# plancherb1/parallel-DDP

Measured on AMD Instinct MI355X. Metric: DDP iterations/sec (Kuka iiwa14 N=128, 8 alphas, 4 shooting segments), higher is better.
Workload: dtype f32; 1 GPU; BASELINE configs[2]: Kuka iiwa14 RBD (n=14,m=7), N=128, 8 alphas x 4 shooting segments, Euler, fp32, joint cost, T=0.5 s, WAFR example inputs + N(0,1e-3) velocity noise; problems_per_gpu=16384, problems_total=16384, hipgraph=True, cost_to_go_slots_written=all, handle_options=library defaults

## Files before the change

parallel-ddp_amd/csrc/pddp_tl.hip:

```cpp
#include <hip/hip_runtime.h>

#include "ab_compact.hpp"
#include "bodies.hpp"
#include "fp_lg.hpp"
#include "fp_pipe.hpp"
#include "tl_launch.hpp"

namespace pddp {

template <typename T> struct TlStagedSink {
    typedef T v4 __attribute__((ext_vector_type(4)));
    T* ds; mutable T* cur; int stride; T* stg; int lane, a, A;
    __device__ __forceinline__ void x(int, const T*) const {}
    __device__ __forceinline__ void u(int, const T*) const {}
    __device__ __forceinline__ void d(int k, const T* v) const { tl_store14(ds + (size_t)k * 14, v); }
    __device__ __forceinline__ void xu(int, const T* xv, const T* uv) const {
        wsync();
        T* rec = stg + lane * 22;
        tl_store14(rec, xv); tl_store7(rec + 14, uv);
        wsync();
        const T* src = stg + (lane - a) * 22 + 4 * a; T* dst = cur - 18 * a;
        const int step = 4 * A;
#pragma unroll
        for (int j = 0; j < 5; j++) *reinterpret_cast<v4*>(dst + step * j) = *reinterpret_cast<const v4*>(src + step * j);
        if (2 * a < A) *reinterpret_cast<v4*>(dst + step * 5) = *reinterpret_cast<const v4*>(src + step * 5);
        cur += stride;
    }
    __device__ __forceinline__ void xu_last(int, const T* xv, const T* uv) const { tl_store14(cur, xv); tl_store7(cur + 14, uv); }
};
constexpr int kFpTlPS = 132;
constexpr int kFpTlMaxPairs = 8;
template <typename T, int V, bool ALL, bool EE = false, bool PC = false>
#ifndef PDDP_FP_TL_MINBLK
#define PDDP_FP_TL_MINBLK 3
#endif
__global__ __launch_bounds__(256, sizeof(T) == 4 && !EE && !ALL && !PC ? PDDP_FP_TL_MINBLK : 2) void k_fp_tl(Buffers<T> b, Dims dm, CostWeights<T> cw, T dt, T grav, int batch) {
    if constexpr (!PC) b.cwt = nullptr;
    constexpr ArmTlModel<T> md = arm_tl_builtin<T>(V);
    constexpr int NX = 14, NU = 7, PS = kFpTlPS;
    const int A = dm.A, M = dm.M, N = dm.N, NBk = dm.NB, per_pb = M * A, total = batch * per_pb;
    const int inst = blockIdx.x * 256 + threadIdx.x;
    if (A < 8 || (64 % A) != 0) {
        if (inst >= total) return;
        const int pb = inst / per_pb, rem = inst - pb * per_pb, seg = rem / A, a_idx = rem - seg * A;
        if (!fp_active<T>(b, dm, pb)) return;
        const T* xcur = b.xb + ((size_t)pb * 2 + b.state[pb].cur) * N * NX;
        if (EE) {
            if (ALL) arm_tl_rollout_segment_ee<T>(md, grav, b, dm, cw, dt, pb, a_idx, seg, xcur, tl_candidate_sink<T>(b, dm, pb, a_idx), true);
            else arm_tl_rollout_segment_ee<T>(md, grav, b, dm, cw, dt, pb, a_idx, seg, xcur, tl_state_sink<T>(b, dm, pb, a_idx), true);
        } else {
            if (ALL) arm_tl_rollout_segment<T>(md, grav, b, dm, cw, dt, pb, a_idx, seg, xcur, tl_candidate_sink<T>(b, dm, pb, a_idx), true);
            else arm_tl_rollout_segment<T>(md, grav, b, dm, cw, dt, pb, a_idx, seg, xcur, tl_state_sink<T>(b, dm, pb, a_idx), true);
        }
        return;
    }
    __shared__ __attribute__((aligned(16))) T stage_all[4 * 2 * kFpTlMaxPairs * PS];
    const int wave = threadIdx.x >> 6, lane = threadIdx.x & 63;
    T* stg = stage_all + wave * (2 * kFpTlMaxPairs * PS);
    const int ppw = 64 / A, npairs = batch * M;
    const int gp0 = (blockIdx.x * 256 + wave * 64) / A;
    if (gp0 >= npairs) return;
    constexpr int J2 = (kFpTlMaxPairs * 56 + 63) / 64, J1 = (kFpTlMaxPairs * 14 + 63) / 64;
    const T* src2[J2]; int dst2[J2], str2[J2];
    const T* src1[J1]; int dst1[J1];
#pragma unroll
    for (int j = 0; j < J2; j++) {
        const int e = lane + 64 * j, q = e / 56, off = e - q * 56;
        int gq = gp0 + (q < ppw ? q : ppw - 1); gq = gq < npairs ? gq : npairs - 1;
        const int pbq = gq / M, k0 = (gq - pbq * M) * NBk;
        const bool isK = off < 49;
        src2[j] = isK ? b.KT + ((size_t)pbq * N + k0) * (NX * NU) + 2 * off
                      : b.xb + (((size_t)pbq * 2 + b.state[pbq].cur) * N + k0) * NX + 2 * (off - 49);
        str2[j] = isK ? NX * NU : NX;
        dst2[j] = (e < ppw * 56) ? q * PS + (isK ? 2 * off : 98 + 2 * (off - 49)) : -1;
    }
#pragma unroll
    for (int j = 0; j < J1; j++) {
        const int e = lane + 64 * j, q = e / 14, off = e - q * 14;
        int gq = gp0 + (q < ppw ? q : ppw - 1); gq = gq < npairs ? gq : npairs - 1;
        const int pbq = gq / M, k0 = (gq - pbq * M) * NBk;
        src1[j] = (off < 7 ? b.ucur : b.du) + ((size_t)pbq * N + k0) * NU + (off < 7 ? off : off - 7);
        dst1[j] = (e < ppw * 14) ? q * PS + 112 + off : -1;
    }
    TlPair<T> pf2[J2]; T pf1[J1];
    auto fetch = [&]() {
#pragma unroll
        for (int j = 0; j < J2; j++) { pf2[j] = *reinterpret_cast<const TlPair<T>*>(src2[j]); src2[j] += str2[j]; }
#pragma unroll
        for (int j = 0; j < J1; j++) { pf1[j] = src1[j][0]; src1[j] += NU; }
    };
    auto park = [&](int buf) {
        T* d = stg + buf * (kFpTlMaxPairs * PS);
#pragma unroll
        for (int j = 0; j < J2; j++) if (dst2[j] >= 0) *reinterpret_cast<TlPair<T>*>(d + dst2[j]) = pf2[j];
#pragma unroll
        for (int j = 0; j < J1; j++) if (dst1[j] >= 0) d[dst1[j]] = pf1[j];
    };
    const int p = lane / A, a_idx = lane - p * A, gp = gp0 + p;
    const int pb = (gp < npairs ? gp : npairs - 1) / M, seg = (gp < npairs ? gp : npairs - 1) - pb * M;
    const bool live = gp < npairs && fp_active<T>(b, dm, pb);
    const T* xcur = b.xb + ((size_t)pb * 2 + b.state[pb].cur) * N * NX;
    constexpr bool REC = PC && !EE;
    constexpr int XGS = REC ? 24 : 16;
    __shared__ __attribute__((aligned(16))) T xg_all[4 * kFpTlMaxPairs * XGS];
    T* xg = xg_all + (wave * kFpTlMaxPairs + p) * XGS;
    if (a_idx == 0) { T t[NX]; tl_load14(t, b.xGoal + (size_t)pb * NX); tl_store14(xg, t); }
    if constexpr (REC) {
        if (a_idx == 0) {
            const CostWeights<T> own = cost_weights_at(b, cw, pb);
            xg[16] = own.Q1; xg[17] = own.Q2; xg[18] = own.R; xg[19] = own.QF1; xg[20] = own.QF2;
        }
    }
    const auto own_cw = [&]() { if constexpr (REC) return cost_weights_joint_row(cw, xg + 16); else return cw; };
    T xt[EE ? NX : 1], acc[EE ? NU : 1];
    int tshift = 0;
    if (EE) {
        tl_load14(xt, b.xTarget + (size_t)pb * NX);
#pragma unroll
        for (int i = 0; i < NU; i++) acc[i] = T(0);
        tshift = b.tshift[pb];
    }
    TlRollout<T> r;
    r.iters = 0;
    const auto csink = tl_candidate_sink<T>(b, dm, pb, a_idx);
    constexpr bool STG = sizeof(T) == 4 && !ALL;
    const auto rsink = tl_run_sink<T>(b, dm, pb, a_idx, seg * NBk);
    const auto ssink = [&]() { if constexpr (STG) return TlStagedSink<T>{rsink.ds, rsink.cur, rsink.stride, stg, lane, a_idx, A}; else return rsink; }();
    if (live) {
        if (ALL) tl_rollout_begin<T>(r, b, dm, pb, a_idx, seg, xcur, csink); else tl_rollout_begin<T>(r, b, dm, pb, a_idx, seg, xcur, ssink);
        if (EE) r.iters = NBk;
    }
    fetch(); park(0);
    wsync();
    for (int k = 0; k < NBk; k++) {
        if (k + 1 < NBk) fetch();
        if (live && k < r.iters) {
            const T* o = stg + (k & 1) * (kFpTlMaxPairs * PS) + p * PS;
            if (EE) {
                if (ALL) tl_rollout_step_ee<T>(r, acc, md, grav, b, dm, cw, dt, k, o, o + 98, o + 112, o + 119, xg, xt, tshift, csink);
                else tl_rollout_step_ee<T>(r, acc, md, grav, b, dm, cw, dt, k, o, o + 98, o + 112, o + 119, xg, xt, tshift, ssink);
            } else {
                if (ALL) tl_rollout_step<T>(r, md, grav, b, dm, own_cw(), dt, k, o, o + 98, o + 112, o + 119, xg, csink);
                else tl_rollout_step<T>(r, md, grav, b, dm, own_cw(), dt, k, o, o + 98, o + 112, o + 119, xg, ssink);
            }
        }
        if (k + 1 < NBk) park((k + 1) & 1);
        wsync();
    }
    if (!live) return;
    if (EE) tl_rollout_end_ee<T>(r, acc, dm);
    else {
        T ucN[NU];
#pragma unroll
        for (int i = 0; i < NU; i++) ucN[i] = b.ucur[((size_t)pb * N + (N - 1)) * NU + i];
        if (ALL) tl_rollout_end<T>(r, dm, own_cw(), ucN, xg, csink); else tl_rollout_end<T>(r, dm, own_cw(), ucN, xg, ssink);
    }
    const size_t slot = (size_t)pb * A + a_idx;
    b.Jpart[slot * M + seg] = r.J; b.dpart[slot * M + seg] = r.sdef;
    b.parts_fresh[pb] = 1;
}

template <int V>
__global__ __launch_bounds__(128, 1) void k_fp_tl2(Buffers<float> b, Dims dm, CostWeights<float> cw, float dt, float grav, int batch) {
    using T = float;
    constexpr ArmTlModel<T> md = arm_tl_builtin<T>(V);
    constexpr int NX = 14, NU = 7, ST = 9, SX = 15;
    __shared__ T s_tau[64 * ST];
    __shared__ T s_x[64 * SX];
    const int wave = __builtin_amdgcn_readfirstlane((int)threadIdx.x >> 6), lane = threadIdx.x & 63;
    const int A = dm.A, M = dm.M, N = dm.N, NBk = dm.NB, total = batch * M * A;
    const int inst_raw = blockIdx.x * 64 + lane, inst = inst_raw < total ? inst_raw : total - 1;
    const int pb = inst / (M * A), rem = inst - pb * (M * A), seg = rem / A, a_idx = rem - seg * A;
    const bool live = inst_raw < total && fp_active<T>(b, dm, pb);
    cw = cost_weights_at(b, cw, pb);
    const int kStart = seg * NBk, iters = (seg < M - 1) ? NBk : NBk - 1;
    const T* xcur = b.xb + ((size_t)pb * 2 + b.state[pb].cur) * N * NX;
    const size_t slot = (size_t)pb * A + a_idx;
    T* xs = b.xs + slot * N * NX; T* us = b.us + slot * N * NU; T* ds = b.ds + slot * N * NX;
    T x[NX];
    if (seg == 0) tl_load14(x, xcur); else tl_load14(x, xs + (size_t)kStart * NX);
    if (wave == 0) {
        const T alpha = b.alpha[a_idx];
        const T* KT = b.KT + (size_t)pb * N * NX * NU; const T* uc = b.ucur + (size_t)pb * N * NU; const T* du = b.du + (size_t)pb * N * NU;
        T xg[NX];
        tl_load14(xg, b.xGoal + (size_t)pb * NX);
        T J = T(0);
        T nK[NX * NU], nxr[NX], nuc[NU], ndu[NU];
        auto fetch = [&](int kn) {
#pragma unroll
            for (int rr = 0; rr < NU; rr++) tl_load14(nK + rr * NX, KT + (size_t)kn * (NX * NU) + rr * NX);
            tl_load14(nxr, xcur + (size_t)kn * NX);
#pragma unroll
            for (int i = 0; i < NU; i++) { nuc[i] = uc[(size_t)kn * NU + i]; ndu[i] = du[(size_t)kn * NU + i]; }
        };
        fetch(kStart);
        for (int k = 0; k < NBk; k++) {
            const int kn = kStart + k;
            const bool act = live && k < iters;
            if (act) {
                T u[NU];
                tl_control_law<T>(u, alpha, ndu, nK, x, nxr, nuc);
                if (k + 1 < NBk) fetch(kn + 1);
#pragma unroll
                for (int i = 0; i < NU; i++) us[(size_t)kn * NU + i] = u[i];
                J += arm_tl_cost<T>(cw, x, u, xg, false);
                ArmTlState<T> st;
                T bias[NU];
                arm_tl_trig<T>(st, x);
                arm_tl_bias<T>(md, grav, st, x + 7, bias);
#pragma unroll
                for (int i = 0; i < NU; i++) s_tau[lane * ST + i] = u[i] - bias[i];
            }
            __syncthreads();
            __syncthreads();
            if (act && k < NBk - 1) {
#pragma unroll
                for (int i = 0; i < NX; i++) x[i] = s_x[lane * SX + i];
            }
        }
        if (live) {
            if (seg == M - 1) {
                T u[NU];
#pragma unroll
                for (int i = 0; i < NU; i++) { u[i] = uc[(size_t)(N - 1) * NU + i]; us[(size_t)(N - 1) * NU + i] = u[i]; }
                J += arm_tl_cost<T>(cw, x, u, xg, true);
            }
            b.Jpart[slot * M + seg] = J;
            b.parts_fresh[pb] = 1;
        }
    } else {
        if (live) tl_store14(xs + (size_t)kStart * NX, x);
        T sdef = T(0);
        for (int k = 0; k < NBk; k++) {
            const int kn = kStart + k;
            const bool act = live && k < iters;
            ArmTlState<T> st;
            if (act) { arm_tl_trig<T>(st, x); arm_tl_factor<T>(md, st); }
            __syncthreads();
            if (act) {
                T qdd[NU], xn[NX];
#pragma unroll
                for (int i = 0; i < NU; i++) qdd[i] = s_tau[lane * ST + i];
                tl_ldl_solve(st, qdd);
#pragma unroll
                for (int i = 0; i < 7; i++) { xn[i] = x[i] + dt * x[7 + i]; xn[7 + i] = x[7 + i] + dt * qdd[i]; }
                if (k < NBk - 1) {
#pragma unroll
                    for (int i = 0; i < NX; i++) { x[i] = xn[i]; s_x[lane * SX + i] = xn[i]; }
                    tl_store14(xs + (size_t)(kn + 1) * NX, xn);
                } else {
                    const int ks = (seg + 1) * NBk;
                    T xnext[NX], e[NX];
                    tl_load14(xnext, xs + (size_t)ks * NX);
#pragma unroll
                    for (int i = 0; i < NX; i++) { e[i] = xn[i] - xnext[i]; sdef += tabs(e[i]); }
                    tl_store14(ds + (size_t)(ks - 1) * NX, e);
                }
            }
            __syncthreads();
        }
        if (live) b.dpart[slot * M + seg] = (seg == M - 1) ? T(0) : sdef;
    }
}
void launch_fp_tl2(hipStream_t s, int variant, const Buffers<float>& b, const Dims& dm, const CostWeights<float>& cw, float dt, float grav, int batch) {
    const unsigned inst = (unsigned)batch * dm.M * dm.A;
    if (variant == 0) hipLaunchKernelGGL((k_fp_tl2<0>), dim3((inst + 63) / 64), dim3(128), 0, s, b, dm, cw, dt, grav, batch);
    else hipLaunchKernelGGL((k_fp_tl2<1>), dim3((inst + 63) / 64), dim3(128), 0, s, b, dm, cw, dt, grav, batch);
}

template <typename T> __device__ __forceinline__ T tl4_fma(T a, T b_, T c) { return __builtin_fma(a, b_, c); }
template <> __device__ __forceinline__ float tl4_fma<float>(float a, float b_, float c) { return __builtin_fmaf(a, b_, c); }
template <typename T, int V, bool EE>
__global__ __launch_bounds__(256, 1) void k_fp_tl4(Buffers<T> b, Dims dm, CostWeights<T> cw, T dt, T grav, int batch, SolverParams sp, int ls_mode, int maps) {
    constexpr int NX = 14, NU = 7;
    __shared__ T ls_J[64], ls_d[64];
    extern __shared__ __attribute__((aligned(16))) unsigned char pipe_lds_raw[];
    const TlPipeLdsT<T> p = tl_pipe_lds(reinterpret_cast<T*>(pipe_lds_raw), true);
    const int wave = __builtin_amdgcn_readfirstlane((int)threadIdx.x >> 6), lane = threadIdx.x & 63;
    if (threadIdx.x < kPipeFlags) p.flag[threadIdx.x] = 0;
    const int A = dm.A, M = dm.M, N = dm.N, NBk = dm.NB, total = batch * M * A;
    const int inst_raw = blockIdx.x * 64 + lane, inst = inst_raw < total ? inst_raw : total - 1;
    const int pb = inst / (M * A), rem = inst - pb * (M * A), seg = rem / A, a_idx = rem - seg * A;
    const bool live = inst_raw < total && fp_active<T>(b, dm, pb);
    cw = cost_weights_at(b, cw, pb);
    const int kStart = seg * NBk;
    const T* xcur = b.xb + ((size_t)pb * 2 + b.state[pb].cur) * N * NX;
    const size_t slot = (size_t)pb * A + a_idx;
    T* xs = b.xs + slot * N * NX; T* us = b.us + slot * N * NU; T* ds = b.ds + slot * N * NX;
    const T alpha = b.alpha[a_idx];
    T x[NX];
    if (!maps) { if (seg == 0) tl_load14(x, xcur); else tl_load14(x, xs + (size_t)kStart * NX); }
    else {
        const int W = M * A, l = rem < NX ? rem : NX - 1;
        const T* dcur = b.dcur + (size_t)pb * N * NX;
        tl_load14(x, xcur + (size_t)kStart * NX);
        T es = T(0), et = T(0);
        auto advance = [&](int sgm, const T* ph, T gam, T dk) {
            T ns = gam, nt = dk;
#pragma unroll
            for (int cc = 0; cc < NX; cc++) { ns = tl4_fma<T>(ph[cc], __shfl(es, cc, W), ns); nt = tl4_fma<T>(ph[cc], __shfl(et, cc, W), nt); }
            es = ns; et = nt;
#pragma unroll
            for (int i = 0; i < NX; i++) {
                const T si = __shfl(es, i, W), ti = __shfl(et, i, W);
                if (seg == sgm + 1) x[i] = x[i] + (ti - alpha * si);
            }
        };
        if (M == 4) {
            T ph[3][NX + 1], dk[3];
#pragma unroll
            for (int sgm = 0; sgm < 3; sgm++) {
                const T* o = b.segmap + ((size_t)pb * 4 + sgm) * 256;
#pragma unroll
                for (int cc = 0; cc <= NX; cc++) ph[sgm][cc] = o[cc * 16 + l];
                dk[sgm] = dcur[(size_t)((sgm + 1) * NBk - 1) * NX + l];
            }
#pragma unroll
            for (int sgm = 0; sgm < 3; sgm++) advance(sgm, ph[sgm], ph[sgm][NX], dk[sgm]);
        } else {
            for (int sgm = 0; sgm < M - 1; sgm++) {
                const T* o = b.segmap + ((size_t)pb * M + sgm) * 256;
                T ph[NX + 1];
#pragma unroll
                for (int cc = 0; cc <= NX; cc++) ph[cc] = o[cc * 16 + l];
                advance(sgm, ph, ph[NX], dcur[(size_t)((sgm + 1) * NBk - 1) * NX + l]);
            }
        }
    }
    __syncthreads();
    if (wave >= 2) { tl_pipe_factor_wave<V>(p, wave - 2, NBk, x, dt, lane); return; }
    if (wave == 0) {
        for (int k = 0; k < NBk; k++) tl_pipe_chain_step<V, true>(p, k, x, (const T*)nullptr, dt, grav, lane);
        return;
    }
    T x0[NX];
#pragma unroll
    for (int i = 0; i < NX; i++) x0[i] = x[i];
    const T* KT = b.KT + (size_t)pb * N * NX * NU; const T* uc = b.ucur + (size_t)pb * N * NU; const T* du = b.du + (size_t)pb * N * NU;
    T xg[NX], goal[6], acc7s[NU];
    int tshift = 0;
    if (EE) {
#pragma unroll
        for (int i = 0; i < 6; i++) goal[i] = b.xGoal[(size_t)pb * NX + i];
        tl_load14(xg, b.xTarget + (size_t)pb * NX);
        tshift = b.tshift[pb];
#pragma unroll
        for (int i = 0; i < NU; i++) acc7s[i] = T(0);
    } else tl_load14(xg, b.xGoal + (size_t)pb * NX);
    T J = T(0), sdef = T(0);
    T nK[NX * NU], nxr[NX], nuc[NU], ndu[NU];
    auto fetch = [&](int kn) {
#pragma unroll
        for (int rr = 0; rr < NU; rr++) tl_load14(nK + rr * NX, KT + (size_t)kn * (NX * NU) + rr * NX);
        tl_load14(nxr, xcur + (size_t)kn * NX);
#pragma unroll
        for (int i = 0; i < NU; i++) { nuc[i] = uc[(size_t)kn * NU + i]; ndu[i] = du[(size_t)kn * NU + i]; }
    };
    fetch(kStart);
    if (live) tl_store14(xs + (size_t)kStart * NX, x);
    const int iters = EE ? NBk : ((seg < M - 1) ? NBk : NBk - 1);
    for (int k = 0; k < NBk; k++) {
        const int kn = kStart + k;
        if (k > 0) {
            T xv[16];
            tl_pipe_wait(p.flag + 0, k);
            tl_pipe_ld<4>(xv, p.xbuf + (((k & 1) * 64) + lane) * kPipeSX);
#pragma unroll
            for (int i = 0; i < NX; i++) x[i] = xv[i];
        }
        T u[8];
        tl_control_law<T>(u, alpha, ndu, nK, x, nxr, nuc);
        u[7] = T(0);
        tl_pipe_st<2>(p.ubuf + (((k & 1) * 64) + lane) * kPipeSU, u);
        tl_pipe_post(p.flag + 1, k + 1);
        if (k + 1 < NBk) fetch(kn + 1);
        if (k > 0 && live) tl_store14(xs + (size_t)kn * NX, x);
        if (live && k < iters) {
#pragma unroll
            for (int i = 0; i < NU; i++) us[(size_t)kn * NU + i] = u[i];
            if (!EE) J += arm_tl_cost<T>(cw, x, u, xg, false);
            else if (k < NBk - 1 || seg == M - 1) {
                constexpr ArmTlModel<T> md = arm_tl_builtin<T>(V);
                ArmTlState<T> st;
                arm_tl_trig<T>(st, x);
                ArmTlFrames<T> fr;
                arm_tl_world_chain<false, T>(md, st.c, st.s, fr);
                T pos[6];
                arm_tl_tool_point<T>(fr, cw.ee_z, tl_ee_rpy_weighted<T>(cw), pos);
#pragma unroll
                for (int ind = 0; ind < NU; ind++) {
                    T cost = T(0);
                    if (ind == 0) cost += ee_term<T>(cw, pos, goal, kn >= N - 1 - tshift);
                    acc7s[ind] += ee_joint_terms<T>(cw, x, u, xg, ind, kn, N, cost);
                }
            }
        }
    }
    T xnext[NX];
    if (maps) {
#pragma unroll
        for (int i = 0; i < NX; i++) xnext[i] = __shfl(x0[i], (lane + A) & 63);
    }
    if (seg < M - 1) {
        tl_pipe_wait(p.flag + 0, NBk);
        if (live) {
            T xi[16];
            tl_pipe_ld<4>(xi, p.xbuf + ((((NBk) & 1) * 64) + lane) * kPipeSX);
            const int ks = (seg + 1) * NBk;
            T e[NX];
            if (!maps) tl_load14(xnext, xs + (size_t)ks * NX);
#pragma unroll
            for (int i = 0; i < NX; i++) { e[i] = xi[i] - xnext[i]; sdef += tabs(e[i]); }
            tl_store14(ds + (size_t)(ks - 1) * NX, e);
        }
    } else if (!EE && live) {
        T u[NU];
#pragma unroll
        for (int i = 0; i < NU; i++) { u[i] = uc[(size_t)(N - 1) * NU + i]; us[(size_t)(N - 1) * NU + i] = u[i]; }
        J += arm_tl_cost<T>(cw, x, u, xg, true);
    }
    if (EE) J = acc7s[0] + acc7s[1] + acc7s[2] + acc7s[3] + acc7s[4] + acc7s[5] + acc7s[6];
    const T dseg = (seg == M - 1) ? T(0) : sdef;
    if (live) {
        b.Jpart[slot * M + seg] = J;
        b.dpart[slot * M + seg] = dseg;
        if (ls_mode < 0) b.parts_fresh[pb] = 1;
    }
    if (ls_mode >= 0) {
        ls_J[lane] = J; ls_d[lane] = dseg;
        wsync();
        const int base = lane - rem;
        if (live && seg == 0) {
            T Jt = T(0), mx = T(0);
            for (int sgm = 0; sgm < M; sgm++) { Jt += ls_J[base + sgm * A + a_idx]; mx = tmax(mx, ls_d[base + sgm * A + a_idx]); }
            b.J[slot] = Jt; b.dmax[slot] = mx;
            ls_J[lane] = Jt; ls_d[lane] = mx;
        }
        wsync();
        if (inst_raw < total && rem == 0) ls_body<T>(b, dm, sp, pb, ls_mode, ls_J + lane, ls_d + lane);
    }
}
template <typename T>
void launch_fp_tl4(hipStream_t s, int variant, const Buffers<T>& b, const Dims& dm, const CostWeights<T>& cw, T dt, T grav, int batch, const SolverParams& sp, int ls_mode, bool maps) {
    const unsigned inst = (unsigned)batch * dm.M * dm.A;
    constexpr int lds = pipe_lds_bytes<T>(true);
    static bool attr_set = false;
    if (!attr_set) {
        hipFuncSetAttribute(reinterpret_cast<const void*>(&k_fp_tl4<T, 0, false>), hipFuncAttributeMaxDynamicSharedMemorySize, lds);
        hipFuncSetAttribute(reinterpret_cast<const void*>(&k_fp_tl4<T, 1, false>), hipFuncAttributeMaxDynamicSharedMemorySize, lds);
        hipFuncSetAttribute(reinterpret_cast<const void*>(&k_fp_tl4<T, 0, true>), hipFuncAttributeMaxDynamicSharedMemorySize, lds);
        hipFuncSetAttribute(reinterpret_cast<const void*>(&k_fp_tl4<T, 1, true>), hipFuncAttributeMaxDynamicSharedMemorySize, lds);
        attr_set = true;
    }
    const dim3 g((inst + 63) / 64), t(256);
    if (cw.ee) {
        if (variant == 0) hipLaunchKernelGGL((k_fp_tl4<T, 0, true>), g, t, lds, s, b, dm, cw, dt, grav, batch, sp, ls_mode, maps ? 1 : 0);
        else hipLaunchKernelGGL((k_fp_tl4<T, 1, true>), g, t, lds, s, b, dm, cw, dt, grav, batch, sp, ls_mode, maps ? 1 : 0);
    } else {
        if (variant == 0) hipLaunchKernelGGL((k_fp_tl4<T, 0, false>), g, t, lds, s, b, dm, cw, dt, grav, batch, sp, ls_mode, maps ? 1 : 0);
        else hipLaunchKernelGGL((k_fp_tl4<T, 1, false>), g, t, lds, s, b, dm, cw, dt, grav, batch, sp, ls_mode, maps ? 1 : 0);
    }
}
template void launch_fp_tl4<float>(hipStream_t, int, const Buffers<float>&, const Dims&, const CostWeights<float>&, float, float, int, const SolverParams&, int, bool);
template void launch_fp_tl4<double>(hipStream_t, int, const Buffers<double>&, const Dims&, const CostWeights<double>&, double, double, int, const SolverParams&, int, bool);

#if defined(__clang__)
#pragma clang fp contract(fast)
#endif
__global__ __launch_bounds__(64) void k_sweep_st(Buffers<float> b, Dims dm, int batch) {
    using L = LgDevice<float>;
    constexpr int NX = 14, NP = 7;
    const int gi = blockIdx.x * kLgPerWave + (threadIdx.x >> 3), pb = gi >> 1, which = gi & 1;
    if (pb >= batch || L::lane() == 7 || !fp_active<float>(b, dm, pb)) return;
    const unsigned pbN = (unsigned)pb * dm.N, oxc = ((unsigned)pb * 2 + b.state[pb].cur) * dm.N * NX;
    const int k_last = (dm.M - 1) * dm.NB - 1, A = dm.A, a0 = which ? (A + 1) / 2 : 0, a1 = which ? A : (A + 1) / 2;
    float eq = 0.f, ev = 0.f;
    constexpr int kDepth = 4;
    float Aq[kDepth][NX], Av[kDepth][NX], cq[kDepth], cv[kDepth];
    const float* add = which ? b.dcur : b.Bdu;
    auto fetch = [&](int slot, int k) {
        const unsigned oA = (pbN + k) * 196, ob = (pbN + k) * 14;
#pragma unroll
        for (int i = 0; i < 14; i++) { Aq[slot][i] = L::gather_at(b.ApBK, oA, [i](int l) { return l + 14 * i; }); Av[slot][i] = L::gather_at(b.ApBK, oA, [i](int l) { return l + 7 + 14 * i; }); }
        cq[slot] = L::gather_at(add, ob, [](int l) { return l; }); cv[slot] = L::gather_at(add, ob, [](int l) { return l + 7; });
    };
    auto step = [&](int slot, int k) {
        float bc[14];
        lg_bcast14<L>(bc, eq, ev);
        float vq = Aq[slot][0] * bc[0], vv = Av[slot][0] * bc[0];
#pragma unroll
        for (int i = 1; i < NX; i++) { vq += Aq[slot][i] * bc[i]; vv += Av[slot][i] * bc[i]; }
        const bool bnd = dm.on_defect_boundary(k);
        if (which == 0 || bnd) { vq += cq[slot]; vv += cv[slot]; }
        eq = vq; ev = vv;
        if (k + kDepth <= k_last) fetch(slot, k + kDepth);
        if (bnd) {
            const float oq = __shfl_xor(eq, 8), ov = __shfl_xor(ev, 8);
            const float sq = which ? oq : eq, sv = which ? ov : ev, tq = which ? eq : oq, tv = which ? ev : ov;
            const float nq = L::gather_at(b.xb, oxc, [k](int l) { return 14 * (k + 1) + l; }), nv = L::gather_at(b.xb, oxc, [k](int l) { return 14 * (k + 1) + l + 7; });
            for (int a = a0; a < a1; a++) {
                const float al = b.alpha[a];
                const unsigned o = (((unsigned)pb * A + a) * dm.N + k + 1) * NX;
                L::scatter_at(b.xs, o, [](int l) { return l; }, nq + (tq - al * sq), true);
                L::scatter_at(b.xs, o, [](int l) { return l + NP; }, nv + (tv - al * sv), true);
            }
        }
    };
#pragma unroll
    for (int j = 0; j < kDepth; j++) if (j <= k_last) fetch(j, j);
    for (int k0 = 0; k0 <= k_last; k0 += kDepth) {
#pragma unroll
        for (int j = 0; j < kDepth; j++) if (k0 + j <= k_last) step(j, k0 + j);
    }
}
#if defined(__clang__)
#pragma clang fp contract(off)
#endif
void launch_sweep_st(hipStream_t s, const Buffers<float>& b, const Dims& dm, int batch) {
    hipLaunchKernelGGL(k_sweep_st, dim3((2 * (unsigned)batch + kLgPerWave - 1) / kLgPerWave), dim3(64), 0, s, b, dm, batch);
}

constexpr int kSweepWgChunk = 96;
typedef float sw4 __attribute__((ext_vector_type(4)));
__device__ __forceinline__ int sw_uniform(int v) { return __builtin_amdgcn_readfirstlane(v); }
__global__ __launch_bounds__(256) __attribute__((amdgpu_waves_per_eu(2, 8))) void k_sweep_wg(Buffers<float> b, Dims dm) {
    extern __shared__ __attribute__((aligned(16))) float sweep_lds[];
    constexpr int NX = 14, SZ = NX * NX;
    const int pb = blockIdx.x;
    if (!fp_active<float>(b, dm, pb)) return;
    const int NBk = dm.NB, nseg = dm.M - 1, N = dm.N;
    if (nseg <= 0) return;
    const int seg_per_chunk = kSweepWgChunk / NBk, chunk = seg_per_chunk * NBk;
    float* F = sweep_lds; float* cB = F + (size_t)chunk * SZ; float* Et = cB + (size_t)chunk * 16 + 16;
    const float* gF = b.ApBK + (size_t)pb * N * SZ; const float* gB = b.Bdu + (size_t)pb * N * NX;
    const float* xcur = b.xb + ((size_t)pb * 2 + b.state[pb].cur) * N * NX; const float* dcur = b.dcur + (size_t)pb * N * NX;
    const int lane = threadIdx.x & 63, g = lane >> 4, c = lane & 15, row0 = 4 * g;
    const int wave = sw_uniform((int)threadIdx.x >> 6);
    const float* pF = F + (c < NX ? c : NX - 1) + NX * row0;
    const float* pC = cB + row0;
    for (int s0 = 0; s0 < nseg; s0 += seg_per_chunk) {
        const int segs = nseg - s0 < seg_per_chunk ? nseg - s0 : seg_per_chunk, k0 = s0 * NBk, cnt = segs * NBk;
        __syncthreads();
        {
            const float4* src = reinterpret_cast<const float4*>(gF + (size_t)k0 * SZ); float4* dst = reinterpret_cast<float4*>(F);
            for (int i = threadIdx.x; i < cnt * (SZ / 4); i += 256) dst[i] = src[i];
            for (int i = threadIdx.x; i < cnt * 16; i += 256) { const int kk = i >> 4, e = i & 15; cB[i] = e < NX ? gB[((size_t)k0 + kk) * NX + e] : 0.f; }
            if (cnt < chunk && threadIdx.x < 2 * NX) F[(size_t)cnt * SZ + threadIdx.x] = 0.f;
        }
        __syncthreads();
        for (int sl = wave; sl < segs; sl += 4) {
            const int kbase = sl * NBk;
            sw4 E;
#pragma unroll
            for (int r = 0; r < 4; r++) E[r] = (row0 + r == c && c < NX) ? 1.f : 0.f;
            for (int j = 0; j < NBk; j++) {
                const int kk = kbase + j;
                sw4 X;
#pragma unroll
                for (int r = 0; r < 4; r++) X[r] = pF[kk * SZ + NX * r];
                const sw4 cv = *reinterpret_cast<const sw4*>(pC + kk * 16);
                sw4 acc;
#pragma unroll
                for (int r = 0; r < 4; r++) acc[r] = c == 14 ? cv[r] : 0.f;
                if (j == NBk - 1) {
#pragma unroll
                    for (int r = 0; r < 4; r++) if (c == 15 && row0 + r < NX) acc[r] = dcur[(size_t)(k0 + kk) * NX + row0 + r];
                }
#pragma unroll
                for (int r = 0; r < 4; r++) acc = __builtin_amdgcn_mfma_f32_16x16x4f32(X[r], E[r], acc, 0, 0, 0);
                E[0] = acc[0]; E[1] = acc[1]; E[2] = g == 3 ? 0.f : acc[2]; E[3] = g == 3 ? 0.f : acc[3];
            }
            float* o = Et + (size_t)(s0 + sl) * 256;
#pragma unroll
            for (int r = 0; r < 4; r++) o[(row0 + r) * 16 + c] = E[r];
        }
    }
    __syncthreads();
    if (wave != 0) return;
    const int l = lane < NX ? lane : NX - 1;
    float es = 0.f, et = 0.f;
    for (int sgm = 0; sgm < nseg; sgm++) {
        const float* o = Et + (size_t)sgm * 256 + l * 16;
        float ns = o[14], nt = o[15];
#pragma unroll
        for (int cc = 0; cc < NX; cc++) {
            const float ph = o[cc];
            ns = __builtin_fmaf(ph, __shfl(es, cc), ns); nt = __builtin_fmaf(ph, __shfl(et, cc), nt);
        }
        es = ns; et = nt;
        if (lane < NX) {
            const int k = (sgm + 1) * NBk - 1;
            const float base = xcur[(size_t)(k + 1) * NX + lane];
            for (int a = 0; a < dm.A; a++) b.xs[(((size_t)pb * dm.A + a) * N + k + 1) * NX + lane] = base + (et - b.alpha[a] * es);
        }
    }
}
static size_t sweep_wg_lds(const Dims& dm) {
    const int chunk = (kSweepWgChunk / dm.NB) * dm.NB;
    return ((size_t)chunk * (14 * 14 + 16) + 16 + (size_t)(dm.M > 1 ? dm.M - 1 : 1) * 256) * sizeof(float);
}
void launch_sweep_wg(hipStream_t s, const Buffers<float>& b, const Dims& dm, int batch) {
    static bool attr_set = false;
    if (!attr_set) { hipFuncSetAttribute(reinterpret_cast<const void*>(&k_sweep_wg), hipFuncAttributeMaxDynamicSharedMemorySize, (kSweepWgChunk * (14 * 14 + 16) + 16 + 15 * 256) * (int)sizeof(float)); attr_set = true; }
    hipLaunchKernelGGL(k_sweep_wg, dim3((unsigned)batch), dim3(256), sweep_wg_lds(dm), s, b, dm);
}

template <typename T>
__global__ __launch_bounds__(256) void k_abc_convert(Buffers<T> b, int knots, int N, T dt, int to_compact) {
    const int i = blockIdx.x * 256 + threadIdx.x;
    if (i >= knots * 21) return;
    const int G = i / 21, col = i - G * 21;
    if (!to_compact && (G % N) == N - 1) return;
    T* full = b.AB + ((size_t)G * 21 + col) * 14;
    T* cmp = b.ABc + abc_index((size_t)G, col, 0);
    if (to_compact) { for (int r = 0; r < 7; r++) cmp[r] = full[7 + r]; }
    else { for (int r = 0; r < 7; r++) { full[r] = tl_AB_const<T>(r, col, dt); full[7 + r] = cmp[r]; } }
}
template <typename T>
void launch_abc_convert(hipStream_t s, const Buffers<T>& b, int knots, int N, T dt, int to_compact) {
    hipLaunchKernelGGL((k_abc_convert<T>), dim3(((unsigned)knots * 21 + 255) / 256), dim3(256), 0, s, b, knots, N, dt, to_compact);
}
template void launch_abc_convert<float>(hipStream_t, const Buffers<float>&, int, int, float, int);
template void launch_abc_convert<double>(hipStream_t, const Buffers<double>&, int, int, double, int);

template <typename T, int V>
__global__ __launch_bounds__(256, 1) void k_plant_eval_tl(T grav, int count, const T* x, const T* u, T* out, int grad) {
    constexpr ArmTlModel<T> md = arm_tl_builtin<T>(V);
    const int i = blockIdx.x * 256 + threadIdx.x;
    if (i >= count) return;
    T xi[14], ui[7], qdd[7];
    for (int e = 0; e < 14; e++) xi[e] = x[(size_t)i * 14 + e];
    for (int e = 0; e < 7; e++) ui[e] = u[(size_t)i * 7 + e];
    ArmTlState<T> st;
    if (grad == 2) {
        ArmTlFrames<T> fr;
        arm_tl_trig<T>(st, xi); arm_tl_world_chain<true, T>(md, st.c, st.s, fr);
        T pos[6], dpos[42];
        arm_tl_tool_point<T>(fr, grav, true, pos); arm_tl_tool_jacobian<T>(fr, grav, dpos);
        for (int e = 0; e < 6; e++) out[(size_t)i * 48 + e] = pos[e];
        for (int e = 0; e < 42; e++) out[(size_t)i * 48 + 6 + e] = dpos[e];
        return;
    }
    arm_tl_dynamics<T>(md, grav, st, qdd, xi, xi + 7, ui);
    if (!grad) { for (int e = 0; e < 7; e++) out[(size_t)i * 7 + e] = qdd[e]; return; }
    T* o = out + (size_t)i * 147;
    arm_tl_gradient<T>(md, grav, st, xi + 7, qdd, [o](int col, int row, T val) { o[7 * col + row] = val; });
}

template <typename T>
void launch_fp_tl(hipStream_t s, int variant, const Buffers<T>& b, const Dims& dm, const CostWeights<T>& cw, T dt, T grav, int batch, int store_candidates) {
    const unsigned inst = (unsigned)batch * dm.M * dm.A;
    const dim3 g((inst + 255) / 256), t(256);
#define PDDP_FP_TL(VV, AL, EEV) do { if (b.cwt) hipLaunchKernelGGL((k_fp_tl<T, VV, AL, EEV, true>), g, t, 0, s, b, dm, cw, dt, grav, batch); \
                                     else hipLaunchKernelGGL((k_fp_tl<T, VV, AL, EEV>), g, t, 0, s, b, dm, cw, dt, grav, batch); } while (0)
    if (cw.ee) {
        if (variant == 0) { if (store_candidates) PDDP_FP_TL(0, true, true); else PDDP_FP_TL(0, false, true); }
        else { if (store_candidates) PDDP_FP_TL(1, true, true); else PDDP_FP_TL(1, false, true); }
    } else {
        if (variant == 0) { if (store_candidates) PDDP_FP_TL(0, true, false); else PDDP_FP_TL(0, false, false); }
        else { if (store_candidates) PDDP_FP_TL(1, true, false); else PDDP_FP_TL(1, false, false); }
    }
#undef PDDP_FP_TL
}
template <typename T>
void launch_plant_eval_tl(hipStream_t s, int variant, T grav, int count, const T* x, const T* u, T* out, int grad) {
    if (variant == 0) hipLaunchKernelGGL((k_plant_eval_tl<T, 0>), dim3((count + 255) / 256), dim3(256), 0, s, grav, count, x, u, out, grad);
    else hipLaunchKernelGGL((k_plant_eval_tl<T, 1>), dim3((count + 255) / 256), dim3(256), 0, s, grav, count, x, u, out, grad);
}
template void launch_fp_tl<float>(hipStream_t, int, const Buffers<float>&, const Dims&, const CostWeights<float>&, float, float, int, int);
template void launch_fp_tl<double>(hipStream_t, int, const Buffers<double>&, const Dims&, const CostWeights<double>&, double, double, int, int);
template void launch_plant_eval_tl<float>(hipStream_t, int, float, int, const float*, const float*, float*, int);
template void launch_plant_eval_tl<double>(hipStream_t, int, double, int, const double*, const double*, double*, int);

}
```

Before: 7.714 million DDP iterations/s.

## Split direct forward-pass kernel and compact per-lane fetch tables into LDS

Moves the fallback path for unsupported alpha counts into its own kernel, so the tiled kernel no longer carries its register cost. The per-lane arrays of prefetch source pointers and destination offsets are replaced by one packed 16-byte descriptor row per lane, kept in LDS, plus a single wave-uniform base pointer. Loads are specialised for A=8. An optional late-fetch mode, enabled when the min-blocks setting is at least 4, drops the second staging buffer and issues the next step's loads after compute. The aim is lower register and LDS pressure and higher occupancy, at the cost of extra LDS reads and an added barrier per step in late mode.

```diff
diff --git a/parallel-ddp_amd/csrc/pddp_tl.hip b/parallel-ddp_amd/csrc/pddp_tl.hip
--- a/parallel-ddp_amd/csrc/pddp_tl.hip
+++ b/parallel-ddp_amd/csrc/pddp_tl.hip
@@ -30,76 +30,90 @@
 };
 constexpr int kFpTlPS = 132;
 constexpr int kFpTlMaxPairs = 8;
-template <typename T, int V, bool ALL, bool EE = false, bool PC = false>
 #ifndef PDDP_FP_TL_MINBLK
 #define PDDP_FP_TL_MINBLK 3
 #endif
-__global__ __launch_bounds__(256, sizeof(T) == 4 && !EE && !ALL && !PC ? PDDP_FP_TL_MINBLK : 2) void k_fp_tl(Buffers<T> b, Dims dm, CostWeights<T> cw, T dt, T grav, int batch) {
+template <typename T, bool ALL, bool EE, bool PC> constexpr int kFpTlMinBlk = sizeof(T) == 4 && !EE && !ALL && !PC ? PDDP_FP_TL_MINBLK : 2;
+template <typename T, bool ALL, bool EE, bool PC> constexpr bool kFpTlLate = kFpTlMinBlk<T, ALL, EE, PC> >= 4;
+template <typename T, int V, bool ALL, bool EE = false, bool PC = false>
+__global__ __launch_bounds__(256, 2) void k_fp_tl_direct(Buffers<T> b, Dims dm, CostWeights<T> cw, T dt, T grav, int batch) {
+    if constexpr (!PC) b.cwt = nullptr;
+    constexpr ArmTlModel<T> md = arm_tl_builtin<T>(V);
+    constexpr int NX = 14;
+    const int A = dm.A, M = dm.M, N = dm.N, per_pb = M * A, total = batch * per_pb;
+    const int inst = blockIdx.x * 256 + threadIdx.x;
+    if (inst >= total) return;
+    const int pb = inst / per_pb, rem = inst - pb * per_pb, seg = rem / A, a_idx = rem - seg * A;
+    if (!fp_active<T>(b, dm, pb)) return;
+    const T* xcur = b.xb + ((size_t)pb * 2 + b.state[pb].cur) * N * NX;
+    if (EE) {
+        if (ALL) arm_tl_rollout_segment_ee<T>(md, grav, b, dm, cw, dt, pb, a_idx, seg, xcur, tl_candidate_sink<T>(b, dm, pb, a_idx), true);
+        else arm_tl_rollout_segment_ee<T>(md, grav, b, dm, cw, dt, pb, a_idx, seg, xcur, tl_state_sink<T>(b, dm, pb, a_idx), true);
+    } else {
+        if (ALL) arm_tl_rollout_segment<T>(md, grav, b, dm, cw, dt, pb, a_idx, seg, xcur, tl_candidate_sink<T>(b, dm, pb, a_idx), true);
+        else arm_tl_rollout_segment<T>(md, grav, b, dm, cw, dt, pb, a_idx, seg, xcur, tl_state_sink<T>(b, dm, pb, a_idx), true);
+    }
+}
+template <typename T, int V, bool ALL, bool EE = false, bool PC = false>
+__global__ __launch_bounds__(256, (kFpTlMinBlk<T, ALL, EE, PC>)) void k_fp_tl(Buffers<T> b, Dims dm, CostWeights<T> cw, T dt, T grav, int batch) {
     if constexpr (!PC) b.cwt = nullptr;
     constexpr ArmTlModel<T> md = arm_tl_builtin<T>(V);
     constexpr int NX = 14, NU = 7, PS = kFpTlPS;
-    const int A = dm.A, M = dm.M, N = dm.N, NBk = dm.NB, per_pb = M * A, total = batch * per_pb;
-    const int inst = blockIdx.x * 256 + threadIdx.x;
-    if (A < 8 || (64 % A) != 0) {
-        if (inst >= total) return;
-        const int pb = inst / per_pb, rem = inst - pb * per_pb, seg = rem / A, a_idx = rem - seg * A;
-        if (!fp_active<T>(b, dm, pb)) return;
-        const T* xcur = b.xb + ((size_t)pb * 2 + b.state[pb].cur) * N * NX;
-        if (EE) {
-            if (ALL) arm_tl_rollout_segment_ee<T>(md, grav, b, dm, cw, dt, pb, a_idx, seg, xcur, tl_candidate_sink<T>(b, dm, pb, a_idx), true);
-            else arm_tl_rollout_segment_ee<T>(md, grav, b, dm, cw, dt, pb, a_idx, seg, xcur, tl_state_sink<T>(b, dm, pb, a_idx), true);
-        } else {
-            if (ALL) arm_tl_rollout_segment<T>(md, grav, b, dm, cw, dt, pb, a_idx, seg, xcur, tl_candidate_sink<T>(b, dm, pb, a_idx), true);
-            else arm_tl_rollout_segment<T>(md, grav, b, dm, cw, dt, pb, a_idx, seg, xcur, tl_state_sink<T>(b, dm, pb, a_idx), true);
-        }
-        return;
-    }
-    __shared__ __attribute__((aligned(16))) T stage_all[4 * 2 * kFpTlMaxPairs * PS];
-    const int wave = threadIdx.x >> 6, lane = threadIdx.x & 63;
-    T* stg = stage_all + wave * (2 * kFpTlMaxPairs * PS);
-    const int ppw = 64 / A, npairs = batch * M;
+    const int A = dm.A, M = dm.M, N = dm.N, NBk = dm.NB;
+    constexpr bool LATE = kFpTlLate<T, ALL, EE, PC>;
+    constexpr int AREA = LATE ? 64 * 22 : 2 * kFpTlMaxPairs * PS, BUF = LATE ? 0 : kFpTlMaxPairs * PS, TBL = 64 * 16 / (int)sizeof(T);
+    __shared__ __attribute__((aligned(16))) T stage_all[4 * (AREA + TBL)];
+    const int wave = __builtin_amdgcn_readfirstlane((int)threadIdx.x >> 6), lane = threadIdx.x & 63;
+    T* stg = stage_all + wave * (AREA + TBL);
+    const int npairs = batch * M;
     const int gp0 = (blockIdx.x * 256 + wave * 64) / A;
     if (gp0 >= npairs) return;
-    constexpr int J2 = (kFpTlMaxPairs * 56 + 63) / 64, J1 = (kFpTlMaxPairs * 14 + 63) / 64;
-    const T* src2[J2]; int dst2[J2], str2[J2];
-    const T* src1[J1]; int dst1[J1];
-#pragma unroll
-    for (int j = 0; j < J2; j++) {
-        const int e = lane + 64 * j, q = e / 56, off = e - q * 56;
-        int gq = gp0 + (q < ppw ? q : ppw - 1); gq = gq < npairs ? gq : npairs - 1;
-        const int pbq = gq / M, k0 = (gq - pbq * M) * NBk;
-        const bool isK = off < 49;
-        src2[j] = isK ? b.KT + ((size_t)pbq * N + k0) * (NX * NU) + 2 * off
-                      : b.xb + (((size_t)pbq * 2 + b.state[pbq].cur) * N + k0) * NX + 2 * (off - 49);
-        str2[j] = isK ? NX * NU : NX;
-        dst2[j] = (e < ppw * 56) ? q * PS + (isK ? 2 * off : 98 + 2 * (off - 49)) : -1;
-    }
-#pragma unroll
-    for (int j = 0; j < J1; j++) {
-        const int e = lane + 64 * j, q = e / 14, off = e - q * 14;
-        int gq = gp0 + (q < ppw ? q : ppw - 1); gq = gq < npairs ? gq : npairs - 1;
-        const int pbq = gq / M, k0 = (gq - pbq * M) * NBk;
-        src1[j] = (off < 7 ? b.ucur : b.du) + ((size_t)pbq * N + k0) * NU + (off < 7 ? off : off - 7);
-        dst1[j] = (e < ppw * 14) ? q * PS + 112 + off : -1;
-    }
-    TlPair<T> pf2[J2]; T pf1[J1];
-    auto fetch = [&]() {
-#pragma unroll
-        for (int j = 0; j < J2; j++) { pf2[j] = *reinterpret_cast<const TlPair<T>*>(src2[j]); src2[j] += str2[j]; }
-#pragma unroll
-        for (int j = 0; j < J1; j++) { pf1[j] = src1[j][0]; src1[j] += NU; }
-    };
-    auto park = [&](int buf) {
-        T* d = stg + buf * (kFpTlMaxPairs * PS);
-#pragma unroll
-        for (int j = 0; j < J2; j++) if (dst2[j] >= 0) *reinterpret_cast<TlPair<T>*>(d + dst2[j]) = pf2[j];
-#pragma unroll
-        for (int j = 0; j < J1; j++) if (dst1[j] >= 0) d[dst1[j]] = pf1[j];
-    };
     const int p = lane / A, a_idx = lane - p * A, gp = gp0 + p;
     const int pb = (gp < npairs ? gp : npairs - 1) / M, seg = (gp < npairs ? gp : npairs - 1) - pb * M;
     const bool live = gp < npairs && fp_active<T>(b, dm, pb);
-    const T* xcur = b.xb + ((size_t)pb * 2 + b.state[pb].cur) * N * NX;
+    const int xsel = b.state[pb].cur;
+    const T* xcur = b.xb + ((size_t)pb * 2 + xsel) * N * NX;
+    typedef unsigned FetchRow __attribute__((ext_vector_type(4)));
+    FetchRow* const row = reinterpret_cast<FetchRow*>(stg + AREA) + lane;
+    const int pb0 = __builtin_amdgcn_readfirstlane(pb);
+    {
+        const int fa = live ? a_idx : 64;
+        const unsigned rk = (unsigned)((pb - pb0) * N + seg * NBk);
+        FetchRow t;
+        t.x = rk * (NX * NU) + 2 * fa; t.y = (unsigned)(((pb - pb0) * 2 + xsel) * N + seg * NBk) * NX + 2 * fa; t.z = rk * NU + fa; t.w = (unsigned)(p * PS + 2 * fa) | (unsigned)fa << 16;
+        *row = t;
+    }
+    const T* const gK = b.KT + (size_t)pb0 * N * (NX * NU); const T* const gX = b.xb + (size_t)pb0 * 2 * N * NX;
+    const T* const gU = b.ucur + (size_t)pb0 * N * NU; const T* const gD = b.du + (size_t)pb0 * N * NU;
+    constexpr int JK = (49 + 7) / 8;
+    TlPair<T> pfK[JK], pfX; T pfU, pfD;
+    auto fetch_as = [&](int k, auto Ac) {
+        const unsigned Aj = Ac;
+        const FetchRow t = *row;
+        const unsigned fa = t.w >> 16;
+        if (fa < Aj) {
+            const T* sK = gK + (size_t)k * (NX * NU) + t.x;
+#pragma unroll
+            for (unsigned j = 0; j < JK; j++) if (Aj * (j + 1) <= 49 || fa + Aj * j < 49) pfK[j] = *reinterpret_cast<const TlPair<T>*>(sK + 2 * Aj * j);
+            if (fa < 7) {
+                pfX = *reinterpret_cast<const TlPair<T>*>(gX + (size_t)k * NX + t.y);
+                pfU = (gU + (size_t)k * NU)[t.z]; pfD = (gD + (size_t)k * NU)[t.z];
+            }
+        }
+    };
+    auto park_as = [&](int buf, auto Ac) {
+        const unsigned Aj = Ac;
+        const FetchRow t = *row;
+        const unsigned fa = t.w >> 16;
+        if (fa < Aj) {
+            T* d = stg + buf * BUF + (t.w & 0xffffu);
+#pragma unroll
+            for (unsigned j = 0; j < JK; j++) if (Aj * (j + 1) <= 49 || fa + Aj * j < 49) *reinterpret_cast<TlPair<T>*>(d + 2 * Aj * j) = pfK[j];
+            if (fa < 7) { *reinterpret_cast<TlPair<T>*>(d + 98) = pfX; d[112 - (int)fa] = pfU; d[119 - (int)fa] = pfD; }
+        }
+    };
+    auto fetch = [&](int k) { if (A == 8) fetch_as(k, std::integral_constant<unsigned, 8>()); else fetch_as(k, (unsigned)A); };
+    auto park = [&](int buf) { if (A == 8) park_as(buf, std::integral_constant<unsigned, 8>()); else park_as(buf, (unsigned)A); };
     constexpr bool REC = PC && !EE;
     constexpr int XGS = REC ? 24 : 16;
     __shared__ __attribute__((aligned(16))) T xg_all[4 * kFpTlMaxPairs * XGS];
@@ -130,12 +144,12 @@
         if (ALL) tl_rollout_begin<T>(r, b, dm, pb, a_idx, seg, xcur, csink); else tl_rollout_begin<T>(r, b, dm, pb, a_idx, seg, xcur, ssink);
         if (EE) r.iters = NBk;
     }
-    fetch(); park(0);
+    fetch(0); park(0);
     wsync();
     for (int k = 0; k < NBk; k++) {
-        if (k + 1 < NBk) fetch();
+        if (!LATE && k + 1 < NBk) fetch(k + 1);
         if (live && k < r.iters) {
-            const T* o = stg + (k & 1) * (kFpTlMaxPairs * PS) + p * PS;
+            const T* o = stg + (k & 1) * BUF + p * PS;
             if (EE) {
                 if (ALL) tl_rollout_step_ee<T>(r, acc, md, grav, b, dm, cw, dt, k, o, o + 98, o + 112, o + 119, xg, xt, tshift, csink);
                 else tl_rollout_step_ee<T>(r, acc, md, grav, b, dm, cw, dt, k, o, o + 98, o + 112, o + 119, xg, xt, tshift, ssink);
@@ -144,6 +158,8 @@
                 else tl_rollout_step<T>(r, md, grav, b, dm, own_cw(), dt, k, o, o + 98, o + 112, o + 119, xg, ssink);
             }
         }
+        if (LATE) wsync();
+        if (LATE && k + 1 < NBk) fetch(k + 1);
         if (k + 1 < NBk) park((k + 1) & 1);
         wsync();
     }
@@ -651,7 +667,10 @@
 void launch_fp_tl(hipStream_t s, int variant, const Buffers<T>& b, const Dims& dm, const CostWeights<T>& cw, T dt, T grav, int batch, int store_candidates) {
     const unsigned inst = (unsigned)batch * dm.M * dm.A;
     const dim3 g((inst + 255) / 256), t(256);
-#define PDDP_FP_TL(VV, AL, EEV) do { if (b.cwt) hipLaunchKernelGGL((k_fp_tl<T, VV, AL, EEV, true>), g, t, 0, s, b, dm, cw, dt, grav, batch); \
+    const bool direct = dm.A < 8 || (64 % dm.A) != 0;
+#define PDDP_FP_TL(VV, AL, EEV) do { if (direct) { if (b.cwt) hipLaunchKernelGGL((k_fp_tl_direct<T, VV, AL, EEV, true>), g, t, 0, s, b, dm, cw, dt, grav, batch); \
+                                                   else hipLaunchKernelGGL((k_fp_tl_direct<T, VV, AL, EEV>), g, t, 0, s, b, dm, cw, dt, grav, batch); } \
+                                     else if (b.cwt) hipLaunchKernelGGL((k_fp_tl<T, VV, AL, EEV, true>), g, t, 0, s, b, dm, cw, dt, grav, batch); \
                                      else hipLaunchKernelGGL((k_fp_tl<T, VV, AL, EEV>), g, t, 0, s, b, dm, cw, dt, grav, batch); } while (0)
     if (cw.ee) {
         if (variant == 0) { if (store_candidates) PDDP_FP_TL(0, true, true); else PDDP_FP_TL(0, false, true); }
```

New measurement: 7.730 million DDP iterations/s, median of 3. About the same (+0.2%).
